# rubenwiersma/deltaconv

Hardware: AMD Instinct MI355X
Metric: point-clouds/sec fwd+bwd, ModelNet40 1024pt k=20, 1/2/4/8 MI355X (higher is better)
Workload: dtype f32; 1 GPU; ModelNet40 classification, 1024 points, k=20, batch=32 per GPU, fwd+bwd+SGD step, train-mode BN/Dropout, HIP-graph replay; global_batch=32, parallelism=dp1

## Files before the change

deltaconv_amd/csrc/nn.hip:

```cpp
#include "common.h"
#include "nn_math.h"
#include "colreduce.h"

namespace {

using namespace dcnn;

using namespace dccol;

template <int V>
struct StatsF {
    const float* h; long ld;
    __device__ void operator()(long r, int c0, double (&t)[2][V]) const {
        const FV<V> x = ldv<V>(h + r * ld + c0);
#pragma unroll
        for (int j = 0; j < V; ++j) { t[0][j] = (double)x.v[j]; t[1][j] = (double)x.v[j] * (double)x.v[j]; }
    }
};
template <int V>
struct BnBwdF {
    const float *dy, *h, *scale, *shift, *mean, *invstd; long lddy, ldh; float slope;
    __device__ void operator()(long r, int c0, double (&t)[2][V]) const {
        const FV<V> g = ldv<V>(dy + r * lddy + c0), x = ldv<V>(h + r * ldh + c0);
#pragma unroll
// ... 107 lines not shown
            gi[j] = (gamma ? gamma[c] : 1.f) * invstd[c]; a1[j] = m1[c]; a2[j] = m2[c];
        }
    }
    __device__ void row(long r, int c0) {
        const FV<V> g = ldv<V>(dy + r * lddy + c0), x = ldv<V>(h + r * ldh + c0);
        FV<V> o;
#pragma unroll
        for (int j = 0; j < V; ++j)
            o.v[j] = bn_bwd_dh(g.v[j], x.v[j], sc[j], sh[j], mu[j], is[j], slope, gi[j], a1[j], a2[j], training);
        stv<V>(dh + r * lddh + c0, o);
    }
};

template <int V>
struct VnApplyBody {
    const float *in, *scale, *shift; float* out; long ld, ldo; int co, combine;
    float sc[V], sh[V];
    __device__ void init(int c0) {
#pragma unroll
        for (int j = 0; j < V; ++j) { sc[j] = scale[c0 + j]; sh[j] = shift[c0 + j]; }
    }
    __device__ void row(long i, int c0) {
        FV<V> yu, yv;
        vn_load_y<V>(in, ld, i, c0, co, combine, yu, yv);
#pragma unroll
        for (int j = 0; j < V; ++j) {
            const float s = vn_scale(vn_norm(yu.v[j], yv.v[j]), sc[j], sh[j]);
            yu.v[j] *= s;
            yv.v[j] *= s;
        }
        stv<V>(out + (2 * i) * ldo + c0, yu);
        stv<V>(out + (2 * i + 1) * ldo + c0, yv);
    }
};

template <int V>
struct VnBwdBody {
    const float *in, *dout, *scale, *shift, *mean, *invstd, *gamma, *m1, *m2; float* din;
    long ld, lddo, lddi; int co, combine, training;
    float sc[V], sh[V], mu[V], is[V], gi[V], a1[V], a2[V];
    __device__ void init(int c0) {
#pragma unroll
        for (int j = 0; j < V; ++j) {
            const int c = c0 + j;
            sc[j] = scale[c]; sh[j] = shift[c]; mu[j] = mean[c]; is[j] = invstd[c];
            gi[j] = (gamma ? gamma[c] : 1.f) * invstd[c]; a1[j] = m1[c]; a2[j] = m2[c];
        }
    }
    __device__ void row(long i, int c0) {
        FV<V> yu, yv, gu, gv;
        vn_load_y<V>(in, ld, i, c0, co, combine, yu, yv);
        const FV<V> du = ldv<V>(dout + (2 * i) * lddo + c0), dv = ldv<V>(dout + (2 * i + 1) * lddo + c0);
#pragma unroll
        for (int j = 0; j < V; ++j)
            vn_bwd_dy(yu.v[j], yv.v[j], du.v[j], dv.v[j], sc[j], sh[j], mu[j], is[j], gi[j], a1[j], a2[j], training,
                      gu.v[j], gv.v[j]);
        if (combine == 2) {
            float eu[2 * V], ev[2 * V];
#pragma unroll
            for (int j = 0; j < V; ++j) {
                eu[2 * j] = gu.v[j]; eu[2 * j + 1] = gv.v[j];
                ev[2 * j] = gv.v[j]; ev[2 * j + 1] = -gu.v[j];
            }
            FV<V> a, b, c, d;
#pragma unroll
            for (int j = 0; j < V; ++j) { a.v[j] = eu[j]; b.v[j] = eu[V + j]; c.v[j] = ev[j]; d.v[j] = ev[V + j]; }
            float* ru = din + (2 * i) * lddi + 2 * c0;
            float* rv = din + (2 * i + 1) * lddi + 2 * c0;
            stv<V>(ru, a); stv<V>(ru + V, b); stv<V>(rv, c); stv<V>(rv + V, d);
            return;
        }
        stv<V>(din + (2 * i) * lddi + c0, gu);
        stv<V>(din + (2 * i + 1) * lddi + c0, gv);
        if (combine) {
            FV<V> ngu;
#pragma unroll
            for (int j = 0; j < V; ++j) ngu.v[j] = -gu.v[j];
            stv<V>(din + (2 * i) * lddi + co + c0, gv);
            stv<V>(din + (2 * i + 1) * lddi + co + c0, ngu);
        }
    }
};

template <int V>
__global__ __launch_bounds__(TPB) void pool_fwd_kernel(const float* __restrict__ h, long ldh, int N, int C,
                                                       const float* __restrict__ scale,
                                                       const float* __restrict__ shift, float slope, int with_mean,
                                                       float* __restrict__ pooled, long ldp, int* __restrict__ argmax) {
    __shared__ float smx[RT][CT * V];
    __shared__ float ssm[RT][CT * V];
    __shared__ int sam[RT][CT * V];
    const int cloud = blockIdx.x;
    const int cgl = threadIdx.x % CT, rl = threadIdx.x / CT;
    const int c0 = (blockIdx.y * CT + cgl) * V;
    float mx[V], sm[V], sc[V], sh[V];
    int am[V];
#pragma unroll
    for (int j = 0; j < V; ++j) {
        mx[j] = -INFINITY; sm[j] = 0.f; am[j] = 0;
        sc[j] = c0 < C ? scale[c0 + j] : 0.f; sh[j] = c0 < C ? shift[c0 + j] : 0.f;
    }
    if (c0 < C) {
        const float* base = h + (long)cloud * N * ldh + c0;
#pragma unroll 8
        for (int r = rl; r < N; r += RT) {
            const FV<V> x = ldv<V>(base + (long)r * ldh);
#pragma unroll
            for (int j = 0; j < V; ++j) {
                const float y = act(fmaf(sc[j], x.v[j], sh[j]), slope);
                sm[j] += y;
                if (y > mx[j]) { mx[j] = y; am[j] = r; }
            }
        }
    }
#pragma unroll
    for (int j = 0; j < V; ++j) { smx[rl][cgl * V + j] = mx[j]; ssm[rl][cgl * V + j] = sm[j]; sam[rl][cgl * V + j] = am[j]; }
    __syncthreads();
    for (int idx = threadIdx.x; idx < CT * V; idx += TPB) {
        const int col = blockIdx.y * CT * V + idx;
        if (col >= C) continue;
        float m = smx[0][idx], t = ssm[0][idx];
        int a = sam[0][idx];
#pragma unroll
        for (int rr = 1; rr < RT; ++rr) {
            const float v = smx[rr][idx];
            const int ar = sam[rr][idx];
            if (v > m || (v == m && ar < a)) { m = v; a = ar; }
            t += ssm[rr][idx];
        }
        pooled[(long)cloud * ldp + col] = m;
        if (with_mean) pooled[(long)cloud * ldp + C + col] = t / (float)N;
        argmax[(long)cloud * C + col] = a;
    }
}

template <int V>
struct PoolDy {
    const float* dp; const int* argmax; long ldp; int N, C, with_mean;
    int cur_b; float dmx[V], dme[V]; int ar[V];
    __device__ void reset() { cur_b = -1; }
    __device__ FV<V> get(long r, int c0) {
        const int b = (int)((unsigned)r / (unsigned)N);
        if (b != cur_b) {
            cur_b = b;
#pragma unroll
            for (int j = 0; j < V; ++j) {
                dmx[j] = dp[(long)b * ldp + c0 + j];
                dme[j] = with_mean ? dp[(long)b * ldp + C + c0 + j] / (float)N : 0.f;
                ar[j] = argmax[(long)b * C + c0 + j];
            }
        }
        const int row = (int)r - b * N;
        FV<V> g;
#pragma unroll
        for (int j = 0; j < V; ++j) g.v[j] = (ar[j] == row ? dmx[j] : 0.f) + dme[j];
        return g;
    }
};
template <int V>
struct PoolBwdF {
    PoolDy<V> dy; const float *h, *scale, *shift, *mean, *invstd; long ldh; float slope; int primed;
    __device__ void operator()(long r, int c0, double (&t)[2][V]) {
        if (!primed) { dy.reset(); primed = 1; }
        const FV<V> g = dy.get(r, c0), x = ldv<V>(h + r * ldh + c0);
#pragma unroll
        for (int j = 0; j < V; ++j) {
            float a, b;
            bn_bwd_terms(g.v[j], x.v[j], scale[c0 + j], shift[c0 + j], mean[c0 + j], invstd[c0 + j], slope, a, b);
            t[0][j] = a; t[1][j] = b;
        }
    }
};
template <int V>
struct PoolBwdBody {
    PoolDy<V> dy; const float *h, *scale, *shift, *mean, *invstd, *gamma, *m1, *m2; float* dh;
    long ldh, lddh; float slope; int training;
    float sc[V], sh[V], mu[V], is[V], gi[V], a1[V], a2[V];
    __device__ void init(int c0) {
        dy.reset();
#pragma unroll
        for (int j = 0; j < V; ++j) {
            const int c = c0 + j;
            sc[j] = scale[c]; sh[j] = shift[c]; mu[j] = mean[c]; is[j] = invstd[c];
            gi[j] = (gamma ? gamma[c] : 1.f) * invstd[c]; a1[j] = m1[c]; a2[j] = m2[c];
        }
    }
    __device__ void row(long r, int c0) {
        const FV<V> g = dy.get(r, c0), x = ldv<V>(h + r * ldh + c0);
        FV<V> o;
#pragma unroll
        for (int j = 0; j < V; ++j)
            o.v[j] = bn_bwd_dh(g.v[j], x.v[j], sc[j], sh[j], mu[j], is[j], slope, gi[j], a1[j], a2[j], training);
        stv<V>(dh + r * lddh + c0, o);
    }
};

template <int V>
struct CloudBiasBody {
    const float *h, *g; float* y; long ldh, ldg, ldy, mx;
    __device__ void init(int) {}
    __device__ void row(long r, int c0) {
        const FV<V> x = ldv<V>(h + r * ldh + c0), b = ldv<V>(g + (r / mx) * ldg + c0);
        FV<V> o;
#pragma unroll
        for (int j = 0; j < V; ++j) o.v[j] = x.v[j] + b.v[j];
        stv<V>(y + r * ldy + c0, o);
    }
};

template <int V>
__global__ __launch_bounds__(TPB) void cloud_colsum_kernel(const float* __restrict__ x, long ldx, long mx, int C, int chunks,
                                                           int rpc, double* __restrict__ partial) {
    __shared__ double sm[RT][CT * V];
    const int cgl = threadIdx.x % CT, rl = threadIdx.x / CT;
    const int c0 = (blockIdx.y * CT + cgl) * V;
    const long cloud = blockIdx.z;
    const long r0 = cloud * mx + (long)blockIdx.x * rpc, r1 = min(r0 + rpc, (cloud + 1) * mx);
    double acc[V];
#pragma unroll
    for (int j = 0; j < V; ++j) acc[j] = 0.0;
    if (c0 < C) {
#pragma unroll 2
        for (long r = r0 + rl; r < r1; r += RT) {
            const FV<V> v = ldv<V>(x + r * ldx + c0);
#pragma unroll
            for (int j = 0; j < V; ++j) acc[j] += (double)v.v[j];
        }
    }
#pragma unroll
    for (int j = 0; j < V; ++j) sm[rl][cgl * V + j] = acc[j];
    __syncthreads();
    for (int cl = threadIdx.x; cl < CT * V; cl += TPB) {
        const int col = blockIdx.y * CT * V + cl;
        if (col < C) {
            double t = 0;
#pragma unroll
            for (int rr = 0; rr < RT; ++rr) t += sm[rr][cl];
            partial[(cloud * C + col) * chunks + blockIdx.x] = t;
        }
    }
}
__global__ __launch_bounds__(64) void cloud_colsum_final_kernel(const double* __restrict__ partial, int chunks, int C,
                                                                float* __restrict__ out, long ldo) {
    const int col = blockIdx.x;
    const long cloud = blockIdx.y;
    const double* p = partial + (cloud * C + col) * chunks;
    double t = 0;
    for (int ch = threadIdx.x; ch < chunks; ch += 64) t += p[ch];
    t = dc_wave_sum(t);
    if (threadIdx.x == 0) out[cloud * ldo + col] = (float)t;
}
inline int cloud_colsum_chunks(long num_clouds, long mx, int C) {
    const long coltiles = dc_cdiv(C, CT * 4);
    const long want = std::max<long>(1, 768 / std::max<long>(1, num_clouds * coltiles));
    return (int)std::max<long>(1, std::min<long>(want, dc_cdiv(mx, RT)));
}

template <int V, class BODY>
void run_tile(BODY body, long R, int C, hipStream_t s) {
    const long coltiles = dc_cdiv(C, CT * V);
#ifndef DC_TILE_BLOCKS
#define DC_TILE_BLOCKS 1024
#endif
    long rpc = (R * coltiles / DC_TILE_BLOCKS + RT - 1) / RT * RT;
    rpc = std::min<long>(std::max<long>(rpc, RT), 1024);
    dim3 grid(dc_cdiv(R, rpc), (unsigned)coltiles);
    hipLaunchKernelGGL((tile_kernel<V, BODY>), grid, dim3(TPB), 0, s, R, C, (int)rpc, body);
}

}

DC_EXPORT size_t dc_bn_workspace_bytes(int64_t rows, int32_t C) { return ws_need(rows, C); }

#define DC_WS_CHECK(name, R, C)                                                   \
    if (!workspace || workspace_bytes < ws_need(R, C)) {                          \
// ... 339 lines not shown
    if (c >= C) return;
    fin.R = count > 0 ? count : (long)(gs[2 * C] + 0.5);
    float* dg = fin.dgamma; float* db = fin.dbeta;
    fin.dgamma = nullptr; fin.dbeta = nullptr;
    fin(c, gs[c], gs[C + c]);
    if (db) db[c] = (float)ls[c];
    if (dg) dg[c] = (float)ls[C + c];
}
}
DC_EXPORT int dc_bn_backward_coefs_from_sums(const double* global_sums, int64_t count, const double* local_sums, int32_t C,
                                             const float* gamma, const float* scale, const float* shift, const float* mean,
                                             const float* invstd, int32_t training, float* dgamma, float* dbeta, float* coefs,
                                             void* stream) {
    DC_REQUIRE(global_sums && local_sums && scale && shift && mean && invstd && coefs, "dc_bn_backward_coefs_from_sums: null pointer");
    DC_REQUIRE(C >= 1, "dc_bn_backward_coefs_from_sums: bad size");
    const BwdCoefFin fin{(long)count, gamma, scale, shift, mean, invstd, training, dgamma, dbeta, coefs, C};
    hipLaunchKernelGGL(bn_bwd_coefs_from_sums_kernel, dim3(dc_cdiv(C, 128)), dim3(128), 0, static_cast<hipStream_t>(stream),
                       global_sums, (long)count, local_sums, C, fin);
    DC_CHECK_LAUNCH("dc_bn_backward_coefs_from_sums");
    return DC_OK;
}

DC_EXPORT int dc_bn_act_backward_apply(const float* dy, int64_t lddy, const float* h, int64_t ldh, int64_t R, int32_t C,
                                       const float* scale, const float* shift, const float* mean, const float* invstd,
                                       const float* gamma, float slope, int32_t training, const float* m1,
                                       const float* m2, float* dh, int64_t lddh, void* stream) {
    DC_REQUIRE(dy && h && scale && shift && mean && invstd && m1 && m2 && dh, "dc_bn_act_backward_apply: null pointer");
    DC_REQUIRE(R >= 1 && C >= 1 && lddy >= C && ldh >= C && lddh >= C, "dc_bn_act_backward_apply: bad size");
    hipStream_t s = static_cast<hipStream_t>(stream);
    if (C % 4 == 0 && lddy % 4 == 0 && ldh % 4 == 0 && lddh % 4 == 0 && al16(dy) && al16(h) && al16(dh))
        run_tile<4>(BnActBwdBody<4>{dy, h, scale, shift, mean, invstd, gamma, m1, m2, dh, (long)lddy, (long)ldh,
                                    (long)lddh, slope, training}, R, C, s);
    else
        run_tile<1>(BnActBwdBody<1>{dy, h, scale, shift, mean, invstd, gamma, m1, m2, dh, (long)lddy, (long)ldh,
                                    (long)lddh, slope, training}, R, C, s);
    DC_CHECK_LAUNCH("dc_bn_act_backward_apply");
    return DC_OK;
}

DC_EXPORT int dc_vn_backward_sums(const float* dout, int64_t lddo, const float* in, int64_t ld, int32_t combine,
                                  int64_t n, int32_t co, const float* scale, const float* shift, const float* mean,
                                  const float* invstd, double* sums, void* workspace, size_t workspace_bytes,
                                  void* stream) {
    DC_REQUIRE(dout && in && scale && shift && mean && invstd && sums, "dc_vn_backward_sums: null pointer");
    DC_REQUIRE(n >= 1 && co >= 1 && lddo >= co && ld >= (combine ? 2 * co : co), "dc_vn_backward_sums: bad size");
    DC_WS_CHECK("dc_vn_backward_sums", n, co)
    hipStream_t s = static_cast<hipStream_t>(stream);
    const Ws w = carve(workspace, n, co);
    const SumsFin fin{sums, co, (double)n};
    if (co % 4 == 0 && ld % 4 == 0 && lddo % 4 == 0 && al16(in) && al16(dout))
        run_colreduce<4>(VnBwdF<4>{in, dout, scale, shift, mean, invstd, (long)ld, (long)lddo, co, combine}, n, co, w, s, fin);
    else
        run_colreduce<1>(VnBwdF<1>{in, dout, scale, shift, mean, invstd, (long)ld, (long)lddo, co, combine}, n, co, w, s, fin);
    DC_CHECK_LAUNCH("dc_vn_backward_sums");
    return DC_OK;
}

DC_EXPORT int dc_vn_backward_apply(const float* dout, int64_t lddo, const float* in, int64_t ld, int32_t combine,
                                   int64_t n, int32_t co, const float* scale, const float* shift, const float* mean,
                                   const float* invstd, const float* gamma, int32_t training, const float* m1,
                                   const float* m2, float* din, int64_t lddi, void* stream) {
    DC_REQUIRE(dout && in && scale && shift && mean && invstd && m1 && m2 && din, "dc_vn_backward_apply: null pointer");
    DC_REQUIRE(n >= 1 && co >= 1 && lddo >= co && ld >= (combine ? 2 * co : co) && lddi >= (combine ? 2 * co : co),
               "dc_vn_backward_apply: bad size");
    hipStream_t s = static_cast<hipStream_t>(stream);
    if (co % 4 == 0 && ld % 4 == 0 && lddo % 4 == 0 && lddi % 4 == 0 && al16(in) && al16(dout) && al16(din))
        run_tile<4>(VnBwdBody<4>{in, dout, scale, shift, mean, invstd, gamma, m1, m2, din, (long)ld, (long)lddo,
                                 (long)lddi, co, combine, training}, n, co, s);
    else
        run_tile<1>(VnBwdBody<1>{in, dout, scale, shift, mean, invstd, gamma, m1, m2, din, (long)ld, (long)lddo,
                                 (long)lddi, co, combine, training}, n, co, s);
    DC_CHECK_LAUNCH("dc_vn_backward_apply");
    return DC_OK;
}

DC_EXPORT int dc_bn_act_pool(const float* h, int64_t ldh, int32_t num_clouds, int32_t N, int32_t C, const float* scale,
                             const float* shift, float slope, int32_t with_mean, float* pooled, int64_t ldp,
                             int32_t* argmax, void* stream) {
    DC_REQUIRE(h && scale && shift && pooled && argmax, "dc_bn_act_pool: null pointer");
    DC_REQUIRE(num_clouds >= 1 && N >= 1 && C >= 1 && ldh >= C && ldp >= (with_mean ? 2 * C : C), "dc_bn_act_pool: bad size");
    hipStream_t s = static_cast<hipStream_t>(stream);
    if (C % 4 == 0 && ldh % 4 == 0 && al16(h))
        hipLaunchKernelGGL(pool_fwd_kernel<4>, dim3(num_clouds, dc_cdiv(C, CT * 4)), dim3(TPB), 0, s, h, (long)ldh, N, C, scale,
                           shift, slope, with_mean, pooled, (long)ldp, argmax);
    else
        hipLaunchKernelGGL(pool_fwd_kernel<1>, dim3(num_clouds, dc_cdiv(C, CT)), dim3(TPB), 0, s, h, (long)ldh, N, C, scale,
                           shift, slope, with_mean, pooled, (long)ldp, argmax);
    DC_CHECK_LAUNCH("dc_bn_act_pool");
    return DC_OK;
}

DC_EXPORT int dc_bn_act_pool_backward(const float* dpooled, int64_t ldp, const int32_t* argmax, const float* h,
                                      int64_t ldh, int32_t num_clouds, int32_t N, int32_t C, const float* scale,
                                      const float* shift, const float* mean, const float* invstd, const float* gamma,
                                      float slope, int32_t with_mean, int32_t training, float* dh, int64_t lddh,
                                      float* dgamma, float* dbeta, void* workspace, size_t workspace_bytes,
                                      void* stream) {
    DC_REQUIRE(dpooled && argmax && h && scale && shift && mean && invstd && dh, "dc_bn_act_pool_backward: null pointer");
    DC_REQUIRE(num_clouds >= 1 && N >= 1 && C >= 1 && ldh >= C && lddh >= C && ldp >= (with_mean ? 2 * C : C),
               "dc_bn_act_pool_backward: bad size");
    const long R = (long)num_clouds * N;
    DC_WS_CHECK("dc_bn_act_pool_backward", R, C)
    hipStream_t s = static_cast<hipStream_t>(stream);
    const Ws w = carve(workspace, R, C);
    const BwdFin fin{R, dgamma, dbeta, w.m1, w.m2};
    const bool v4 = C % 4 == 0 && ldh % 4 == 0 && lddh % 4 == 0 && al16(h) && al16(dh);
    DC_REQUIRE(R < 2147483647L, "dc_bn_act_pool_backward: too many rows");
    if (v4) {
        PoolBwdF<4> f{};
        f.dy.dp = dpooled; f.dy.argmax = argmax; f.dy.ldp = ldp; f.dy.N = N; f.dy.C = C; f.dy.with_mean = with_mean;
        f.h = h; f.scale = scale; f.shift = shift; f.mean = mean; f.invstd = invstd; f.ldh = ldh; f.slope = slope; f.primed = 0;
        run_colreduce<4>(f, R, C, w, s, fin);
        PoolBwdBody<4> b{};
        b.dy = f.dy; b.h = h; b.scale = scale; b.shift = shift; b.mean = mean; b.invstd = invstd; b.gamma = gamma;
        b.m1 = w.m1; b.m2 = w.m2; b.dh = dh; b.ldh = ldh; b.lddh = lddh; b.slope = slope; b.training = training;
        run_tile<4>(b, R, C, s);
    } else {
        PoolBwdF<1> f{};
        f.dy.dp = dpooled; f.dy.argmax = argmax; f.dy.ldp = ldp; f.dy.N = N; f.dy.C = C; f.dy.with_mean = with_mean;
        f.h = h; f.scale = scale; f.shift = shift; f.mean = mean; f.invstd = invstd; f.ldh = ldh; f.slope = slope; f.primed = 0;
        run_colreduce<1>(f, R, C, w, s, fin);
        PoolBwdBody<1> b{};
        b.dy = f.dy; b.h = h; b.scale = scale; b.shift = shift; b.mean = mean; b.invstd = invstd; b.gamma = gamma;
        b.m1 = w.m1; b.m2 = w.m2; b.dh = dh; b.ldh = ldh; b.lddh = lddh; b.slope = slope; b.training = training;
        run_tile<1>(b, R, C, s);
    }
    DC_CHECK_LAUNCH("dc_bn_act_pool_backward");
    return DC_OK;
}
```

deltaconv_amd/csrc/nn_math.h:

```cpp
#pragma once
#include "point_math.h"

namespace dcnn {

constexpr float VEC_EPS = 1e-8f;

DC_HD float act(float z, float slope) { return z > 0.f ? z : slope * z; }
DC_HD float dact(float z, float slope) { return z > 0.f ? 1.f : slope; }

DC_HD void bn_bwd_terms(float dy, float h, float scale, float shift, float mean, float invstd, float slope,
                        float& dz, float& dz_xhat) {
    const float z = fmaf(scale, h, shift);
    dz = dy * dact(z, slope);
    dz_xhat = dz * ((h - mean) * invstd);
}
DC_HD float bn_bwd_dh(float dy, float h, float scale, float shift, float mean, float invstd, float slope,
                      float gi , float m1 , float m2 , int training) {
    const float z = fmaf(scale, h, shift);
    const float dz = dy * dact(z, slope);
    if (!training) return scale * dz;
    const float xhat = (h - mean) * invstd;
    return gi * (dz - m1 - xhat * m2);
}

DC_HD void vn_combine(float pu, float qu, float pv, float qv, float& yu, float& yv) {
    yu = pu - qv;
    yv = pv + qu;
}
DC_HD float vn_norm(float yu, float yv) { return sqrtf(fmaf(yu, yu, yv * yv)); }

DC_HD float vn_scale(float n, float scale, float shift) {
    const float z = fmaf(scale, n, shift);
    return (z > 0.f ? z : 0.f) / fmaxf(n, VEC_EPS);
}

DC_HD void vn_bwd_terms(float yu, float yv, float du, float dv, float scale, float shift, float mean, float invstd,
                        float& dz, float& dz_nhat) {
    const float n = vn_norm(yu, yv);
    const float z = fmaf(scale, n, shift);
    const float gs = yu * du + yv * dv;
    dz = z > 0.f ? gs / fmaxf(n, VEC_EPS) : 0.f;
    dz_nhat = dz * ((n - mean) * invstd);
}
DC_HD void vn_bwd_dy(float yu, float yv, float du, float dv, float scale, float shift, float mean, float invstd,
                     float gi, float m1, float m2, int training, float& dyu, float& dyv) {
    const float n = vn_norm(yu, yv);
    const float nc = fmaxf(n, VEC_EPS);
    const float z = fmaf(scale, n, shift);
    const float r = z > 0.f ? z : 0.f;
    const float s = r / nc;
    const float gs = yu * du + yv * dv;
    const float dz = z > 0.f ? gs / nc : 0.f;
    float dn = training ? gi * (dz - m1 - ((n - mean) * invstd) * m2) : scale * dz;
    if (n > VEC_EPS) dn -= gs * r / (nc * nc);
    const float w = n > 0.f ? dn / n : 0.f;
    dyu = fmaf(du, s, w * yu);
    dyv = fmaf(dv, s, w * yv);
}

struct U4 {
    unsigned x, y, z, w;
};
DC_HD unsigned mulhi32(unsigned a, unsigned b) { return (unsigned)(((unsigned long long)a * (unsigned long long)b) >> 32); }
DC_HD U4 philox4x32_10(U4 c, unsigned k0, unsigned k1) {
    for (int r = 0; r < 10; ++r) {
        const unsigned hi0 = mulhi32(0xD2511F53u, c.x), lo0 = 0xD2511F53u * c.x;
        const unsigned hi1 = mulhi32(0xCD9E8D57u, c.z), lo1 = 0xCD9E8D57u * c.z;
        c = U4{hi1 ^ c.y ^ k0, lo1, hi0 ^ c.w ^ k1, lo0};
        k0 += 0x9E3779B9u;
        k1 += 0xBB67AE85u;
    }
    return c;
}
DC_HD bool dropout_keep(unsigned seed, long long step, unsigned salt, unsigned element, float p) {
    const U4 r = philox4x32_10(U4{element, salt, (unsigned)step, (unsigned)((unsigned long long)step >> 32)}, seed, 0x64726F70u);
    return (float)(r.x >> 8) * (1.0f / 16777216.0f) >= p;
}

}
```

deltaconv_amd/nn/fused.py:

```python
import contextlib
import ctypes
import os
import threading

import torch
import torch.nn.functional as F

from .._lib import lib, require_gpu


def _c(t):
    return t if (t is None or (t.dtype == torch.float32 and t.is_contiguous())) else t.contiguous().float()


def _ws(rows, c, device):
    nbytes = lib.raw("dc_bn_workspace_bytes")(rows, c)
    return torch.empty((nbytes + 7) // 8, dtype=torch.float64, device=device), nbytes


_PENDING, _DEFER = [], [0]


def bump_counter(bn):
    if getattr(bn.running_mean, "_dc_eval_coeffs", None) is not None:
# ... 1019 lines not shown
        raise ValueError(f"cloud_bias: h {tuple(h.shape)} against g {tuple(g.shape)} x {mx} rows")
    return _CloudBias.apply(h, _c(g), int(mx))


class _SplitCols(torch.autograd.Function):

    @staticmethod
    def forward(ctx, w, p):
        ctx.cfg = (tuple(w.shape), p)
        return w[:, :p], w[:, p:]

    @staticmethod
    def backward(ctx, da, db):
        (r, c), p = ctx.cfg
        src = da if da is not None else db
        if src is None:
            return None, None
        dw = torch.empty(r, c, dtype=src.dtype, device=src.device)
        pairs = []
        for d, blk in ((da, dw[:, :p]), (db, dw[:, p:])):
            if d is None:
                blk.zero_()
            else:
                pairs.append((d if d.stride(-1) == 1 else d.contiguous(), blk))
        from .. import _ops
        _ops.copy_many(pairs)
        return dw, None


def split_cols(w, p):
    return _SplitCols.apply(w, int(p))


class _LinearBNAct(torch.autograd.Function):

    @staticmethod
    def forward(ctx, x, w, gamma, beta, bn, slope, residual):
        h, coef, use_batch = linear_stats(x, w, bn, gamma, beta)
        r, c = h.shape
        y = torch.empty_like(h)
        res = _c(residual)
        lib.call("dc_bn_act", h, r, c, c, coef[2], coef[3], slope, res, c, y, c)
        ctx.save_for_backward(x, w, h, coef, gamma)
        ctx.cfg = (use_batch, slope, gamma is not None, beta is not None, residual is not None)
        return y

    @staticmethod
    def backward(ctx, dy):
        x, w, h, coef, gamma = ctx.saved_tensors
        training, slope, has_g, has_b, has_res = ctx.cfg
        dy = _c(dy)
        dw, dgamma, dbeta, dx = bn_block_backward(dy, dy.stride(0), x, h, coef, training, gamma, slope, w,
                                                  want_dinp=ctx.needs_input_grad[0])
        return (dx, dw, dgamma if has_g else None, dbeta if has_b else None, None, None, (dy if has_res else None))


def _seed32():
    s = int(torch.initial_seed())
    import torch.distributed as dist
    if dist.is_available() and dist.is_initialized():
        s ^= (dist.get_rank() + 1) * 0x9E3779B1
    return (s ^ (s >> 31)) & 0x7fffffff


USE_ROWBLOCK_DROPOUT = True


def rowblock_dropout_ok(x, lin, bn, residual=None):
    return (USE_ROWBLOCK_DROPOUT and lin.bias is None and residual is None and _rowblock_ok(x, lin.weight) and bn.training
            and bn.track_running_stats and bn.num_batches_tracked is not None and bn.num_batches_tracked.is_cuda)


def linear_bn_act(x, lin, bn, slope, residual=None, dropout=None):
    if dropout is not None:
        assert rowblock_dropout_ok(x, lin, bn, residual)
        return _RowBlock.apply(x, lin.weight, bn.weight, bn.bias, bn, float(slope), (float(dropout[0]), int(dropout[1])))
    if lin.bias is None and residual is None and _rowblock_ok(x, lin.weight):
        return _RowBlock.apply(x, lin.weight, bn.weight, bn.bias, bn, float(slope))
    if lin.bias is None and x.dim() == 2 and x.is_cuda and x.dtype == torch.float32:
        return _LinearBNAct.apply(x, lin.weight, bn.weight, bn.bias, bn, float(slope), residual)
    return bn_act(linear(x, lin.weight, lin.bias), bn, slope, residual)


def _pool_forward(h, coef, slope, num_clouds, n_per, with_mean):
    c = h.shape[1]
    width = 2 * c if with_mean else c
    pooled = torch.empty(num_clouds, width, dtype=torch.float32, device=h.device)
    arg = torch.empty(num_clouds, c, dtype=torch.int32, device=h.device)
    lib.call("dc_bn_act_pool", h, c, num_clouds, n_per, c, coef[2], coef[3], slope, int(with_mean), pooled, width, arg)
    return pooled, arg


def _pool_backward(dpooled, arg, h, coef, gamma, cfg):
    training, slope, num_clouds, n_per, with_mean, has_g, has_b = cfg
    dpooled = _c(dpooled)
    r, c = h.shape
    dh = torch.empty_like(h)
    dgamma, dbeta = _dgamma_dbeta(c, h.device, has_g, has_b)
    ws, nb = _ws(r, c, h.device)
    lib.call("dc_bn_act_pool_backward", dpooled, dpooled.shape[1], arg, h, c, num_clouds, n_per, c, coef[2], coef[3],
             coef[0], coef[1], gamma, slope, int(with_mean), int(training), dh, c, dgamma, dbeta, ws, nb)
    return dh, dgamma, dbeta


class _LinearBNActPool(torch.autograd.Function):

    @staticmethod
    def forward(ctx, x, w, gamma, beta, bn, slope, num_clouds, n_per, with_mean):
        h, coef, use_batch = linear_stats(x, w, bn, gamma, beta)
        pooled, arg = _pool_forward(h, coef, slope, num_clouds, n_per, with_mean)
        ctx.save_for_backward(x, w, h, coef, gamma, arg)
        ctx.cfg = (use_batch, slope, num_clouds, n_per, with_mean, gamma is not None, beta is not None)
        return pooled

    @staticmethod
    def backward(ctx, dpooled):
        x, w, h, coef, gamma, arg = ctx.saved_tensors
        dh, dgamma, dbeta = _pool_backward(dpooled, arg, h, coef, gamma, ctx.cfg)
        dw, dx = linear_grads(dh, x, w, need_dx=ctx.needs_input_grad[0], need_dw=ctx.needs_input_grad[1])
        return dx, dw, dgamma, dbeta, None, None, None, None, None


def linear_bn_act_pool(x, lin, bn, slope, num_clouds, n_per, with_mean):
    require_gpu()
    return _LinearBNActPool.apply(x, lin.weight, bn.weight, bn.bias, bn, float(slope), num_clouds, n_per, with_mean)


class _BNActPool(torch.autograd.Function):

    @staticmethod
    def forward(ctx, h, gamma, beta, rm, rv, use_batch_stats, momentum, eps, slope, num_clouds, n_per, with_mean):
        h = _c(h)
        r, c = h.shape
        dev = h.device
        coef = torch.empty(4, c, dtype=torch.float32, device=dev)
        if use_batch_stats:
            ws, nb = _ws(r, c, dev)
            lib.call("dc_bn_stats", h, r, c, c, gamma, beta, eps, momentum, rm, rv, coef[0], coef[1], coef[2],
                     coef[3], ws, nb)
        else:
            coef = eval_coeffs(gamma, beta, rm, rv, eps, c)
        pooled, arg = _pool_forward(h, coef, slope, num_clouds, n_per, with_mean)
        ctx.save_for_backward(h, coef, gamma, arg)
        ctx.cfg = (use_batch_stats, slope, num_clouds, n_per, with_mean, gamma is not None, beta is not None)
        return pooled

    @staticmethod
    def backward(ctx, dpooled):
        h, coef, gamma, arg = ctx.saved_tensors
        dh, dgamma, dbeta = _pool_backward(dpooled, arg, h, coef, gamma, ctx.cfg)
        return dh, dgamma, dbeta, None, None, None, None, None, None, None, None, None


def bn_act_pool(h, bn, slope, num_clouds, n_per, with_mean):
    require_gpu()
    use_batch, mom, rm, rv, eps = bn_mode(bn, h.shape[0])
    return _BNActPool.apply(h, bn.weight, bn.bias, rm, rv, use_batch, mom, eps, float(slope), num_clouds, n_per, with_mean)
```

include/deltaconv_hip.h:

```cpp
#ifndef DELTACONV_HIP_H
#define DELTACONV_HIP_H
#include <stddef.h>
#include <stdint.h>

#ifdef __cplusplus
extern "C" {
#endif

#define DC_OK 0
#define DC_ERR_ARG (-1)
#define DC_ERR_LAUNCH (-2)
#define DC_ERR_WORKSPACE (-3)
#define DC_FPS_MAX_POINTS (16384)

int32_t dc_version(void);
const char* dc_last_error(void);
int dc_set_option(int32_t key, int32_t value);

int dc_finalisers_begin(void);
int dc_finaliser_defer_next(void);
int dc_gemm_defer_next(void);
int dc_finalisers_end(int32_t discard, void* stream);

int dc_stamp_buffer(uint64_t* buf, int32_t slots);
// ... 226 lines not shown
int dc_bn_sums(const float* h, int64_t R, int32_t C, int64_t ldh, double* sums, void* workspace,
               size_t workspace_bytes, void* stream);
int dc_vn_sums(const float* in, int64_t n, int32_t co, int64_t ld, int32_t combine, double* sums, void* workspace,
               size_t workspace_bytes, void* stream);
int dc_bn_coeffs_from_sums(const double* sums, int64_t count, int32_t C, const float* gamma, const float* beta,
                           float eps, float momentum, float* running_mean, float* running_var, float* mean,
                           float* invstd, float* scale, float* shift, void* stream);
int dc_bn_act_backward_sums(const float* dy, int64_t lddy, const float* h, int64_t ldh, int64_t R, int32_t C,
                            const float* scale, const float* shift, const float* mean, const float* invstd,
                            float slope, double* sums, void* workspace, size_t workspace_bytes, void* stream);
int dc_sync_means(const double* sums, int32_t C, float* m1, float* m2, float* dgamma, float* dbeta, void* stream);
int dc_bn_act_backward_apply(const float* dy, int64_t lddy, const float* h, int64_t ldh, int64_t R, int32_t C,
                             const float* scale, const float* shift, const float* mean, const float* invstd,
                             const float* gamma, float slope, int32_t training, const float* m1, const float* m2,
                             float* dh, int64_t lddh, void* stream);
int dc_vn_backward_sums(const float* dout, int64_t lddo, const float* in, int64_t ld, int32_t combine, int64_t n,
                        int32_t co, const float* scale, const float* shift, const float* mean, const float* invstd,
                        double* sums, void* workspace, size_t workspace_bytes, void* stream);
int dc_vn_backward_apply(const float* dout, int64_t lddo, const float* in, int64_t ld, int32_t combine, int64_t n,
                         int32_t co, const float* scale, const float* shift, const float* mean, const float* invstd,
                         const float* gamma, int32_t training, const float* m1, const float* m2, float* din,
                         int64_t lddi, void* stream);

int dc_presplit_weights(const int64_t* table, const int32_t* chunk_start, int32_t n_entries, int32_t total_chunks, void* stream);
int dc_gemm_next_b_planes(const void* weight, const void* planes, int64_t plane_elems, int64_t ld, int32_t transposed);

int dc_linear_forward(const float* X, int64_t ldx, const float* W, int64_t ldw, int64_t M, int32_t N, int32_t K,
                      float* Y, int64_t ldy, int32_t tile, void* stream);
int dc_linear_backward_input(const float* dY, int64_t lddy, const float* W, int64_t ldw, int64_t M, int32_t N,
                             int32_t K, float* dX, int64_t lddx, int32_t accumulate, int32_t tile, void* stream);
size_t dc_linear_stats_workspace_bytes(int64_t M, int32_t N, int32_t K, int32_t tile);
int dc_linear_bn_stats_forward(const float* X, int64_t ldx, const float* W, int64_t ldw, int64_t M, int32_t N,
                               int32_t K, float* Y, int64_t ldy, const float* gamma, const float* beta, float eps,
                               float momentum, float* running_mean, float* running_var, float* mean, float* invstd,
                               float* scale, float* shift, int32_t tile, void* workspace, size_t workspace_bytes,
                               void* stream);
int dc_linear_vn_stats_forward(const float* V, int64_t ldv, const float* Wst, int64_t ldw, int64_t n, int32_t co,
                               int32_t K, float* PQ, int64_t ldpq, int32_t interleaved, const float* gamma,
                               const float* beta, float eps,
                               float momentum, float* running_mean, float* running_var, float* mean, float* invstd,
                               float* scale, float* shift, int32_t tile, void* workspace, size_t workspace_bytes,
                               void* stream);

int dc_linear_bn_sums_forward(const float* X, int64_t ldx, const float* W, int64_t ldw, int64_t M, int32_t N, int32_t K,
                              float* Y, int64_t ldy, double* sums, int32_t tile, void* workspace, size_t workspace_bytes,
                              void* stream);
int dc_linear_vn_sums_forward(const float* V, int64_t ldv, const float* Wst, int64_t ldw, int64_t n, int32_t co, int32_t K,
                              float* PQ, int64_t ldpq, int32_t interleaved, double* sums, int32_t tile, void* workspace,
                              size_t workspace_bytes, void* stream);

int dc_bn_act_backward_reduce(const float* dy, int64_t lddy, const float* h, int64_t ldh, int64_t R, int32_t C,
                              const float* scale, const float* shift, const float* mean, const float* invstd,
                              const float* gamma, float slope, int32_t training, float* dgamma, float* dbeta,
                              float* coefs, void* workspace, size_t workspace_bytes, void* stream);
int dc_bn_backward_coefs_from_sums(const double* global_sums, int64_t count, const double* local_sums, int32_t C,
                                   const float* gamma, const float* scale, const float* shift, const float* mean,
                                   const float* invstd, int32_t training, float* dgamma, float* dbeta, float* coefs,
                                   void* stream);
int dc_linear_bn_backward_input(const float* dy, int64_t lddy, const float* h, int64_t ldh, const float* coefs,
                                float slope, const float* W, int64_t ldw, int64_t M, int32_t N, int32_t K, float* dX,
                                int64_t lddx, int32_t accumulate, int32_t tile, void* stream);
int dc_linear_bn_backward_weight(const float* dy, int64_t lddy, const float* h, int64_t ldh, const float* coefs,
                                 float slope, const float* X, int64_t ldx, int64_t R, int32_t N, int32_t K, float* dW,
                                 int64_t lddw, int32_t accumulate, void* workspace, size_t workspace_bytes,
                                 void* stream);
int dc_linear_bn_backward_weight_slabs(const float* dy, int64_t lddy, const float* h, int64_t ldh, const float* coefs,
                                       float slope, const float* X, int64_t ldx, int64_t R, int32_t N, int32_t K,
                                       void* workspace, size_t workspace_bytes, int32_t* slabs, void* stream);

int dc_cloud_bias_add(const float* h, int64_t ldh, const float* g, int64_t ldg, int64_t n, int32_t C, int64_t mx, float* y,
                      int64_t ldy, void* stream);
size_t dc_cloud_colsum_workspace_bytes(int32_t num_clouds, int64_t mx, int32_t C);
int dc_cloud_colsum(const float* x, int64_t ldx, int32_t num_clouds, int64_t mx, int32_t C, float* out, int64_t ldo,
                    void* workspace, size_t workspace_bytes, void* stream);

int dc_bn_act_pool(const float* h, int64_t ldh, int32_t num_clouds, int32_t N, int32_t C, const float* scale,
                   const float* shift, float slope, int32_t with_mean, float* pooled, int64_t ldp, int32_t* argmax,
                   void* stream);
int dc_bn_act_pool_backward(const float* dpooled, int64_t ldp, const int32_t* argmax, const float* h, int64_t ldh,
                            int32_t num_clouds, int32_t N, int32_t C, const float* scale, const float* shift,
                            const float* mean, const float* invstd, const float* gamma, float slope,
                            int32_t with_mean, int32_t training, float* dh, int64_t lddh, float* dgamma, float* dbeta,
                            void* workspace, size_t workspace_bytes, void* stream);

size_t dc_ce_loss_workspace_bytes(int64_t num_rows);
int dc_ce_loss(const float* logits, int64_t ld_logits, const int64_t* labels, int64_t num_rows, int32_t num_classes,
               float smoothing, float* loss, float* dlogits, int64_t ld_dlogits, void* workspace,
               size_t workspace_bytes, void* stream);

int32_t dc_rowblock_max_rows(void);
int dc_rowblock_forward(const float* X, int64_t ldx, const float* W, int64_t ldw, const float* bias, int32_t M, int32_t N,
                        int32_t K, const float* gamma, const float* beta, float eps, float momentum, float* running_mean,
                        float* running_var, int32_t mode, float slope, float* H, int64_t ldh, float* coef, float* Y,
                        int64_t ldy, void* stream);
int dc_rowblock_backward(const float* dY, int64_t lddy, const float* H, int64_t ldh, const float* coef, const float* gamma,
                         float slope, int32_t mode, const float* X, int64_t ldx, int32_t M, int32_t N, int32_t K, float* dW,
                         int64_t lddw, float* dbias, float* dgamma, float* dbeta, float* dH, int64_t lddh, void* stream);
int dc_rowblock_forward_dropout(const float* X, int64_t ldx, const float* W, int64_t ldw, int32_t M, int32_t N, int32_t K,
                                const float* gamma, const float* beta, float eps, float momentum, float* running_mean,
                                float* running_var, int32_t mode, float slope, float* H, int64_t ldh, float* coef, float* Y,
                                int64_t ldy, float p, int32_t seed, const int64_t* step, int32_t salt, uint8_t* mask,
                                void* stream);
int dc_rowblock_backward_dropout(const float* dY, int64_t lddy, const float* H, int64_t ldh, const float* coef,
                                 const float* gamma, float slope, int32_t mode, const float* X, int64_t ldx, int32_t M,
                                 int32_t N, int32_t K, float* dW, int64_t lddw, float* dgamma, float* dbeta, float* dH,
                                 int64_t lddh, const uint8_t* mask, float p, void* stream);

int dc_sgd_step(const int64_t* params, const int64_t* grads, const int64_t* bufs, const int64_t* numel, int32_t count,
                const float* lr, float momentum, float weight_decay, void* stream);
int dc_adam_step(const int64_t* params, const int64_t* grads, const int64_t* exp_avgs, const int64_t* exp_avg_sqs,
                 const int64_t* numel, int32_t count, const float* lr, float* step, int32_t* ticket, double beta1, double beta2,
                 float eps, float weight_decay, void* stream);
int dc_copy_many(const int64_t* srcs, const int64_t* dsts, const int64_t* ld_src, const int64_t* ld_dst, const int32_t* rows,
                 const int32_t* cols, int32_t count, void* stream);

int dc_batch_assemble(const float* store_pos, const float* store_norm, const float* store_x, int32_t F,
                      const int64_t* store_y_point, const int64_t* store_y_cloud, const float* store_category, int32_t Cc,
                      const int64_t* store_ptr, int64_t S, const int64_t* idx, int32_t B, int64_t Nt, int32_t max_cloud,
                      const int32_t* op_codes, const float* op_params, int32_t n_ops, int64_t seed, int64_t step, float* pos,
                      float* norm, float* x, int64_t* batch, int32_t* ptr, int64_t* y, float* category, void* stream);

int dc_eval_metrics(const float* logits, int64_t ld_logits, float* votes, const int64_t* y, const int32_t* ptr, int32_t B,
                    int64_t Nt, int32_t P, const float* category, int32_t Cc, const int32_t* part_start,
                    const int32_t* part_count, int64_t* pred, double* iou, int32_t* hit, int32_t* cnt, int32_t* ignored,
                    void* stream);

size_t dc_geodesic_fps_workspace_bytes(int64_t N);
int dc_geodesic_fps_batch(const void* pos, int32_t pos_is_f64, const int64_t* ptr, int32_t B, int32_t max_cloud_size,
                          int32_t n_samples, const int32_t* start, int32_t* out, void* workspace, size_t workspace_bytes,
                          void* stream);

size_t dc_mesh_sample_workspace_bytes(int64_t F_total);
int32_t dc_mesh_scan_faces(void);
int dc_mesh_sample(const float* vert, const int32_t* face, const int64_t* vptr, const int64_t* fptr, int32_t B,
                   int64_t first_mesh_index, int32_t num, int64_t seed, int64_t round, const int64_t* y_vert,
                   float* pos, float* norm, int64_t* y, int32_t* face_id, int64_t* total,
                   void* workspace, size_t workspace_bytes, void* stream);

int dc_knn_cross(const float* query, const int64_t* qptr, const float* ref, const int64_t* rptr, int32_t B,
                 int64_t max_query_cloud, int32_t k, int32_t* idx, float* d2, void* stream);
int dc_knn_interpolate(const float* x, int64_t ldx, int32_t C, const int64_t* qptr, const int64_t* rptr, int32_t B,
                       int64_t max_query_cloud, int32_t k, const int32_t* idx, const float* d2, float* out, int64_t ldo,
                       void* stream);

#ifdef __cplusplus
}
#endif
#endif
```

Baseline: 11300 clouds/s.

## Precompute per-cloud pooling moments in forward to skip backward column reduction

The fused BN+activation+pool forward kernel now also accumulates per-cloud, per-channel counts of positive pre-activations, split sums of inputs, and the input value at the argmax. In backward, a small per-channel kernel turns these into dgamma/dbeta and the BN mean terms in closed form. The full-size column reduction pass over h is replaced by a single elementwise dh pass. The cost is double-precision accumulation and extra shared memory in the forward kernel, plus extra saved tensors.

```diff
diff --git a/deltaconv_amd/csrc/nn.hip b/deltaconv_amd/csrc/nn.hip
--- a/deltaconv_amd/csrc/nn.hip
+++ b/deltaconv_amd/csrc/nn.hip
@@ -213,22 +213,31 @@
     }
 };
 
-template <int V>
+struct PoolMoments {
+    int* npos; double* spos; double* sneg; float* harg;
+};
+template <int V, bool MOM = false>
 __global__ __launch_bounds__(TPB) void pool_fwd_kernel(const float* __restrict__ h, long ldh, int N, int C,
                                                        const float* __restrict__ scale,
                                                        const float* __restrict__ shift, float slope, int with_mean,
-                                                       float* __restrict__ pooled, long ldp, int* __restrict__ argmax) {
+                                                       float* __restrict__ pooled, long ldp, int* __restrict__ argmax,
+                                                       PoolMoments mo) {
     __shared__ float smx[RT][CT * V];
     __shared__ float ssm[RT][CT * V];
     __shared__ int sam[RT][CT * V];
+    __shared__ int snp[MOM ? RT : 1][CT * V];
+    __shared__ double ssp[MOM ? RT : 1][CT * V];
+    __shared__ double ssa[MOM ? RT : 1][CT * V];
     const int cloud = blockIdx.x;
     const int cgl = threadIdx.x % CT, rl = threadIdx.x / CT;
     const int c0 = (blockIdx.y * CT + cgl) * V;
     float mx[V], sm[V], sc[V], sh[V];
-    int am[V];
+    int am[V], np[V];
+    double sp[V], sa[V];
 #pragma unroll
     for (int j = 0; j < V; ++j) {
         mx[j] = -INFINITY; sm[j] = 0.f; am[j] = 0;
+        np[j] = 0; sp[j] = 0.0; sa[j] = 0.0;
         sc[j] = c0 < C ? scale[c0 + j] : 0.f; sh[j] = c0 < C ? shift[c0 + j] : 0.f;
     }
     if (c0 < C) {
@@ -238,14 +247,25 @@
             const FV<V> x = ldv<V>(base + (long)r * ldh);
 #pragma unroll
             for (int j = 0; j < V; ++j) {
-                const float y = act(fmaf(sc[j], x.v[j], sh[j]), slope);
+                const float z = fmaf(sc[j], x.v[j], sh[j]);
+                const float y = act(z, slope);
                 sm[j] += y;
+                if constexpr (MOM) {
+                    const bool pos = act_pos(z);
+                    np[j] += pos ? 1 : 0;
+                    sp[j] += (double)(pos ? x.v[j] : 0.f);
+                    sa[j] += (double)x.v[j];
+                }
                 if (y > mx[j]) { mx[j] = y; am[j] = r; }
             }
         }
     }
 #pragma unroll
     for (int j = 0; j < V; ++j) { smx[rl][cgl * V + j] = mx[j]; ssm[rl][cgl * V + j] = sm[j]; sam[rl][cgl * V + j] = am[j]; }
+    if constexpr (MOM) {
+#pragma unroll
+        for (int j = 0; j < V; ++j) { snp[rl][cgl * V + j] = np[j]; ssp[rl][cgl * V + j] = sp[j]; ssa[rl][cgl * V + j] = sa[j]; }
+    }
     __syncthreads();
     for (int idx = threadIdx.x; idx < CT * V; idx += TPB) {
         const int col = blockIdx.y * CT * V + idx;
@@ -262,6 +282,16 @@
         pooled[(long)cloud * ldp + col] = m;
         if (with_mean) pooled[(long)cloud * ldp + C + col] = t / (float)N;
         argmax[(long)cloud * C + col] = a;
+        if constexpr (MOM) {
+            int n = 0;
+            double p = 0.0, q = 0.0;
+#pragma unroll
+            for (int rr = 0; rr < RT; ++rr) { n += snp[rr][idx]; p += ssp[rr][idx]; q += ssa[rr][idx]; }
+            mo.npos[(long)cloud * C + col] = n;
+            mo.spos[(long)cloud * C + col] = p;
+            mo.sneg[(long)cloud * C + col] = q - p;
+            mo.harg[(long)cloud * C + col] = h[((long)cloud * N + a) * ldh + col];
+        }
     }
 }
 
@@ -322,6 +352,67 @@
 #pragma unroll
         for (int j = 0; j < V; ++j)
             o.v[j] = bn_bwd_dh(g.v[j], x.v[j], sc[j], sh[j], mu[j], is[j], slope, gi[j], a1[j], a2[j], training);
+        stv<V>(dh + r * lddh + c0, o);
+    }
+};
+
+struct PoolSums {
+    const float *dp; long ldp; const int* npos; const double *spos, *sneg; const float *harg, *scale, *shift, *mean, *invstd;
+    float slope; int B, N, C, with_mean; float *dgamma, *dbeta; double* means;
+};
+__global__ __launch_bounds__(64) void pool_bwd_sums_kernel(PoolSums a) {
+    const int c = blockIdx.x;
+    const double mu = (double)a.mean[c], is = (double)a.invstd[c], slp = (double)a.slope;
+    const float sc = a.scale[c], sh = a.shift[c];
+    double t0 = 0.0, t1 = 0.0;
+    for (int b = threadIdx.x; b < a.B; b += 64) {
+        const long bc = (long)b * a.C + c;
+        const int np = a.npos[bc], nn = a.N - np;
+        const double sp = a.spos[bc], sn = a.sneg[bc];
+        const float dmx = a.dp[(long)b * a.ldp + c];
+        const float dme = a.with_mean ? a.dp[(long)b * a.ldp + a.C + c] / (float)a.N : 0.f;
+        const float ha = a.harg[bc];
+        const double A1 = (double)np + slp * (double)nn;
+        const double Ax = ((sp - (double)np * mu) + slp * (sn - (double)nn * mu)) * is;
+        const double da = (double)dact(fmaf(sc, ha, sh), a.slope);
+        const double xa = ((double)ha - mu) * is;
+        t0 += (double)dme * A1 + (double)dmx * da;
+        t1 += (double)dme * Ax + (double)dmx * da * xa;
+    }
+    t0 = dc_wave_sum(t0);
+    t1 = dc_wave_sum(t1);
+    if (threadIdx.x == 0) {
+        const double R = (double)a.B * (double)a.N;
+        if (a.dbeta) a.dbeta[c] = (float)t0;
+        if (a.dgamma) a.dgamma[c] = (float)t1;
+        a.means[c] = t0 / R;
+        a.means[a.C + c] = t1 / R;
+    }
+}
+template <int V>
+struct PoolBwdBodyD {
+    PoolDy<V> dy; const float *h, *scale, *shift, *mean, *invstd, *gamma; const double* means; float* dh;
+    long ldh, lddh; float slope; int C;
+    float sc[V], sh[V]; double gp[V], gn[V], k1[V], k0[V];
+    __device__ void init(int c0) {
+        dy.reset();
+#pragma unroll
+        for (int j = 0; j < V; ++j) {
+            const int c = c0 + j;
+            const double is = (double)invstd[c], gi = (double)(gamma ? gamma[c] : 1.f) * is, m2is = means[C + c] * is;
+            sc[j] = scale[c]; sh[j] = shift[c];
+            gp[j] = gi; gn[j] = gi * (double)slope;
+            k1[j] = -gi * m2is; k0[j] = gi * (m2is * (double)mean[c] - means[c]);
+        }
+    }
+    __device__ void row(long r, int c0) {
+        const FV<V> g = dy.get(r, c0), x = ldv<V>(h + r * ldh + c0);
+        FV<V> o;
+#pragma unroll
+        for (int j = 0; j < V; ++j) {
+            const double gd = act_pos(fmaf(sc[j], x.v[j], sh[j])) ? gp[j] : gn[j];
+            o.v[j] = (float)fma(gd, (double)g.v[j], fma(k1[j], (double)x.v[j], k0[j]));
+        }
         stv<V>(dh + r * lddh + c0, o);
     }
 };
@@ -827,11 +918,23 @@
     hipStream_t s = static_cast<hipStream_t>(stream);
     if (C % 4 == 0 && ldh % 4 == 0 && al16(h))
         hipLaunchKernelGGL(pool_fwd_kernel<4>, dim3(num_clouds, dc_cdiv(C, CT * 4)), dim3(TPB), 0, s, h, (long)ldh, N, C, scale,
-                           shift, slope, with_mean, pooled, (long)ldp, argmax);
+                           shift, slope, with_mean, pooled, (long)ldp, argmax, PoolMoments{});
     else
         hipLaunchKernelGGL(pool_fwd_kernel<1>, dim3(num_clouds, dc_cdiv(C, CT)), dim3(TPB), 0, s, h, (long)ldh, N, C, scale,
-                           shift, slope, with_mean, pooled, (long)ldp, argmax);
+                           shift, slope, with_mean, pooled, (long)ldp, argmax, PoolMoments{});
     DC_CHECK_LAUNCH("dc_bn_act_pool");
+    return DC_OK;
+}
+
+DC_EXPORT int dc_bn_act_pool_moments(const float* h, int64_t ldh, int32_t num_clouds, int32_t N, int32_t C, const float* scale,
+                                     const float* shift, float slope, int32_t with_mean, float* pooled, int64_t ldp,
+                                     int32_t* argmax, int32_t* npos, double* spos, double* sneg, float* harg, void* stream) {
+    DC_REQUIRE(h && scale && shift && pooled && argmax && npos && spos && sneg && harg, "dc_bn_act_pool_moments: null pointer");
+    DC_REQUIRE(num_clouds >= 1 && N >= 1 && C >= 1 && ldh >= C && ldp >= (with_mean ? 2 * C : C), "dc_bn_act_pool_moments: bad size");
+    DC_REQUIRE(C % 4 == 0 && ldh % 4 == 0 && al16(h), "dc_bn_act_pool_moments: rows of h must be 16-byte aligned, C % 4 == 0");
+    hipLaunchKernelGGL((pool_fwd_kernel<4, true>), dim3(num_clouds, dc_cdiv(C, CT * 4)), dim3(TPB), 0, static_cast<hipStream_t>(stream),
+                       h, (long)ldh, N, C, scale, shift, slope, with_mean, pooled, (long)ldp, argmax, PoolMoments{npos, spos, sneg, harg});
+    DC_CHECK_LAUNCH("dc_bn_act_pool_moments");
     return DC_OK;
 }
 
@@ -873,3 +976,30 @@
     DC_CHECK_LAUNCH("dc_bn_act_pool_backward");
     return DC_OK;
 }
+
+DC_EXPORT int dc_bn_act_pool_backward_moments(const float* dpooled, int64_t ldp, const int32_t* argmax, const int32_t* npos,
+                                              const double* spos, const double* sneg, const float* harg, const float* h,
+                                              int64_t ldh, int32_t num_clouds, int32_t N, int32_t C, const float* scale,
+                                              const float* shift, const float* mean, const float* invstd, const float* gamma,
+                                              float slope, int32_t with_mean, float* dh, int64_t lddh, float* dgamma,
+                                              float* dbeta, double* means, void* stream) {
+    DC_REQUIRE(dpooled && argmax && npos && spos && sneg && harg && h && scale && shift && mean && invstd && dh && means,
+               "dc_bn_act_pool_backward_moments: null pointer");
+    DC_REQUIRE(num_clouds >= 1 && N >= 1 && C >= 1 && ldh >= C && lddh >= C && ldp >= (with_mean ? 2 * C : C),
+               "dc_bn_act_pool_backward_moments: bad size");
+    DC_REQUIRE(C % 4 == 0 && ldh % 4 == 0 && lddh % 4 == 0 && al16(h) && al16(dh),
+               "dc_bn_act_pool_backward_moments: rows of h and dh must be 16-byte aligned, C % 4 == 0");
+    const long R = (long)num_clouds * N;
+    DC_REQUIRE(R < 2147483647L, "dc_bn_act_pool_backward_moments: too many rows");
+    hipStream_t s = static_cast<hipStream_t>(stream);
+    const PoolSums sums{dpooled, (long)ldp, npos, spos, sneg, harg, scale, shift, mean, invstd, slope, num_clouds, N, C, with_mean,
+                        dgamma, dbeta, means};
+    hipLaunchKernelGGL(pool_bwd_sums_kernel, dim3(C), dim3(64), 0, s, sums);
+    PoolBwdBodyD<4> b{};
+    b.dy.dp = dpooled; b.dy.argmax = argmax; b.dy.ldp = ldp; b.dy.N = N; b.dy.C = C; b.dy.with_mean = with_mean;
+    b.h = h; b.scale = scale; b.shift = shift; b.mean = mean; b.invstd = invstd; b.gamma = gamma; b.means = means;
+    b.dh = dh; b.ldh = ldh; b.lddh = lddh; b.slope = slope; b.C = C;
+    run_tile<4>(b, R, C, s);
+    DC_CHECK_LAUNCH("dc_bn_act_pool_backward_moments");
+    return DC_OK;
+}
diff --git a/deltaconv_amd/csrc/nn_math.h b/deltaconv_amd/csrc/nn_math.h
--- a/deltaconv_amd/csrc/nn_math.h
+++ b/deltaconv_amd/csrc/nn_math.h
@@ -6,7 +6,8 @@
 constexpr float VEC_EPS = 1e-8f;
 
 DC_HD float act(float z, float slope) { return z > 0.f ? z : slope * z; }
-DC_HD float dact(float z, float slope) { return z > 0.f ? 1.f : slope; }
+DC_HD bool act_pos(float z) { return z > 0.f; }
+DC_HD float dact(float z, float slope) { return act_pos(z) ? 1.f : slope; }
 
 DC_HD void bn_bwd_terms(float dy, float h, float scale, float shift, float mean, float invstd, float slope,
                         float& dz, float& dz_xhat) {
diff --git a/deltaconv_amd/nn/fused.py b/deltaconv_amd/nn/fused.py
--- a/deltaconv_amd/nn/fused.py
+++ b/deltaconv_amd/nn/fused.py
@@ -1125,21 +1125,42 @@
     return bn_act(linear(x, lin.weight, lin.bias), bn, slope, residual)
 
 
-def _pool_forward(h, coef, slope, num_clouds, n_per, with_mean):
+USE_POOL_MOMENTS = [os.environ.get("DC_POOL_MOMENTS", "1") != "0"]
+
+
+def _pool_moments_ok(h, use_batch):
+    return bool(USE_POOL_MOMENTS[0] and use_batch and group_of(use_batch) is None and h.shape[1] % 4 == 0
+                and h.data_ptr() % 16 == 0)
+
+
+def _pool_forward(h, coef, slope, num_clouds, n_per, with_mean, moments=False):
     c = h.shape[1]
     width = 2 * c if with_mean else c
     pooled = torch.empty(num_clouds, width, dtype=torch.float32, device=h.device)
     arg = torch.empty(num_clouds, c, dtype=torch.int32, device=h.device)
+    if moments:
+        npos = torch.empty(num_clouds, c, dtype=torch.int32, device=h.device)
+        sums = torch.empty(2, num_clouds, c, dtype=torch.float64, device=h.device)
+        harg = torch.empty(num_clouds, c, dtype=torch.float32, device=h.device)
+        lib.call("dc_bn_act_pool_moments", h, c, num_clouds, n_per, c, coef[2], coef[3], slope, int(with_mean), pooled, width, arg,
+                 npos, sums[0], sums[1], harg)
+        return pooled, arg, (npos, sums, harg)
     lib.call("dc_bn_act_pool", h, c, num_clouds, n_per, c, coef[2], coef[3], slope, int(with_mean), pooled, width, arg)
-    return pooled, arg
-
-
-def _pool_backward(dpooled, arg, h, coef, gamma, cfg):
+    return pooled, arg, ()
+
+
+def _pool_backward(dpooled, arg, h, coef, gamma, cfg, moments=()):
     training, slope, num_clouds, n_per, with_mean, has_g, has_b = cfg
     dpooled = _c(dpooled)
     r, c = h.shape
     dh = torch.empty_like(h)
     dgamma, dbeta = _dgamma_dbeta(c, h.device, has_g, has_b)
+    if moments and training and dh.data_ptr() % 16 == 0:
+        npos, sums, harg = moments
+        means = torch.empty(2, c, dtype=torch.float64, device=h.device)
+        lib.call("dc_bn_act_pool_backward_moments", dpooled, dpooled.shape[1], arg, npos, sums[0], sums[1], harg, h, c, num_clouds,
+                 n_per, c, coef[2], coef[3], coef[0], coef[1], gamma, slope, int(with_mean), dh, c, dgamma, dbeta, means)
+        return dh, dgamma, dbeta
     ws, nb = _ws(r, c, h.device)
     lib.call("dc_bn_act_pool_backward", dpooled, dpooled.shape[1], arg, h, c, num_clouds, n_per, c, coef[2], coef[3],
              coef[0], coef[1], gamma, slope, int(with_mean), int(training), dh, c, dgamma, dbeta, ws, nb)
@@ -1151,15 +1172,15 @@
     @staticmethod
     def forward(ctx, x, w, gamma, beta, bn, slope, num_clouds, n_per, with_mean):
         h, coef, use_batch = linear_stats(x, w, bn, gamma, beta)
-        pooled, arg = _pool_forward(h, coef, slope, num_clouds, n_per, with_mean)
-        ctx.save_for_backward(x, w, h, coef, gamma, arg)
+        pooled, arg, mom = _pool_forward(h, coef, slope, num_clouds, n_per, with_mean, _pool_moments_ok(h, use_batch))
+        ctx.save_for_backward(x, w, h, coef, gamma, arg, *mom)
         ctx.cfg = (use_batch, slope, num_clouds, n_per, with_mean, gamma is not None, beta is not None)
         return pooled
 
     @staticmethod
     def backward(ctx, dpooled):
-        x, w, h, coef, gamma, arg = ctx.saved_tensors
-        dh, dgamma, dbeta = _pool_backward(dpooled, arg, h, coef, gamma, ctx.cfg)
+        x, w, h, coef, gamma, arg, *mom = ctx.saved_tensors
+        dh, dgamma, dbeta = _pool_backward(dpooled, arg, h, coef, gamma, ctx.cfg, mom)
         dw, dx = linear_grads(dh, x, w, need_dx=ctx.needs_input_grad[0], need_dw=ctx.needs_input_grad[1])
         return dx, dw, dgamma, dbeta, None, None, None, None, None
 
@@ -1183,15 +1204,15 @@
                      coef[3], ws, nb)
         else:
             coef = eval_coeffs(gamma, beta, rm, rv, eps, c)
-        pooled, arg = _pool_forward(h, coef, slope, num_clouds, n_per, with_mean)
-        ctx.save_for_backward(h, coef, gamma, arg)
+        pooled, arg, mom = _pool_forward(h, coef, slope, num_clouds, n_per, with_mean, _pool_moments_ok(h, use_batch_stats))
+        ctx.save_for_backward(h, coef, gamma, arg, *mom)
         ctx.cfg = (use_batch_stats, slope, num_clouds, n_per, with_mean, gamma is not None, beta is not None)
         return pooled
 
     @staticmethod
     def backward(ctx, dpooled):
-        h, coef, gamma, arg = ctx.saved_tensors
-        dh, dgamma, dbeta = _pool_backward(dpooled, arg, h, coef, gamma, ctx.cfg)
+        h, coef, gamma, arg, *mom = ctx.saved_tensors
+        dh, dgamma, dbeta = _pool_backward(dpooled, arg, h, coef, gamma, ctx.cfg, mom)
         return dh, dgamma, dbeta, None, None, None, None, None, None, None, None, None
 
 
diff --git a/include/deltaconv_hip.h b/include/deltaconv_hip.h
--- a/include/deltaconv_hip.h
+++ b/include/deltaconv_hip.h
@@ -332,6 +332,15 @@
                             const float* mean, const float* invstd, const float* gamma, float slope,
                             int32_t with_mean, int32_t training, float* dh, int64_t lddh, float* dgamma, float* dbeta,
                             void* workspace, size_t workspace_bytes, void* stream);
+int dc_bn_act_pool_moments(const float* h, int64_t ldh, int32_t num_clouds, int32_t N, int32_t C, const float* scale,
+                           const float* shift, float slope, int32_t with_mean, float* pooled, int64_t ldp, int32_t* argmax,
+                           int32_t* npos, double* spos, double* sneg, float* harg, void* stream);
+int dc_bn_act_pool_backward_moments(const float* dpooled, int64_t ldp, const int32_t* argmax, const int32_t* npos,
+                                    const double* spos, const double* sneg, const float* harg, const float* h, int64_t ldh,
+                                    int32_t num_clouds, int32_t N, int32_t C, const float* scale, const float* shift,
+                                    const float* mean, const float* invstd, const float* gamma, float slope,
+                                    int32_t with_mean, float* dh, int64_t lddh, float* dgamma, float* dbeta, double* means,
+                                    void* stream);
 
 size_t dc_ce_loss_workspace_bytes(int64_t num_rows);
 int dc_ce_loss(const float* logits, int64_t ld_logits, const int64_t* labels, int64_t num_rows, int32_t num_classes,
```

After: 11380 clouds/s, median of 5. No clear change (+0.7%).
